# hucsmn/suffix_array

Hardware: AMD Instinct MI355X
Metric: input MB/s indexed (SA build) (higher is better)
Workload: dtype u8; 1 GPU; c3_english_256m: 268435456 bytes per GPU, seed base + rank, one independent text per GPU; n_bytes=268435456, sigma=57, symbols_per_key=13, refinement_rounds=9, text_rounds=0, radix_passes=25, unresolved_after_initial_sort=199000237

## Files before the change

### suffix_array_amd/csrc/host/pipeline.hpp

```cpp
#pragma once
#include "support.hpp"
#include "tuning.hpp"
#include "pool.hpp"
#include "sort.hpp"
#include "readback.hpp"

#include <functional>

namespace sa {

static inline Tuning env_tuning() { return Tuning::from_env(N_SORT_VARIANTS, N_SORT32_VARIANTS, N_OS_SHAPES64, N_OS_SHAPES32); }
static inline Tuning route_tuning()
{
    const Tuning tn = env_tuning();
    g_posted_off = tn.no_posted_readback;
    return tn;
}

constexpr size_t GRAM_MAX_ENTRIES = (size_t)1 << 24;
static_assert(GROUP_CAP_MAX == GS_CAP, "Tuning clamps SA_AMD_GROUP_CAP to the kernel's cap");

struct Workspace {
    uint64_t *keysA, *keysB, *keysC;
    uint32_t *valsA, *valsB, *isa, *U0, *U1, *G0, *G1;
// ... 154 lines not shown
                            const Tuning &tn, bool trace)
{
    KeyParams &P = *Pp;
    const uint64_t se = P.sigma;
    const uint64_t cap = (uint64_t)((size_t)n < GRAM_MAX_ENTRIES ? (size_t)n : GRAM_MAX_ENTRIES);
    int g = 0;
    uint64_t S = 1;
    for (int t = 1; t <= 8; ++t) {
        if (S * se > cap) break;
        S *= se; g = t;
        if (tn.gram_g >= 2 && g == tn.gram_g) break;
    }
    if (g < 2) return SA_AMD_OK;
    uint64_t top = 1;
    for (int t = 0; t + 1 < g; ++t) top *= se;
    const int64_t gtiles = ceil_div((int64_t)S, GT_TILE);
    HIP_TRY(hipMemsetAsync(w.gram_flags, 0, (size_t)S, st));
    PROF(KC_MISC, n, st, hipLaunchKernelGGL((k_gram_mark), dim3((unsigned)ceil_div(ceil_div(n, KB_TILE), GM_TPW)), dim3(KB_THREADS), 0, st, dT, n, P, g,
                                            (uint32_t)top, w.gram_flags));
    PROF(KC_MISC, (int64_t)S, st, hipLaunchKernelGGL((k_gram_count), dim3((unsigned)gtiles), dim3(GT_THREADS), 0, st,
                                            (const uint8_t *)w.gram_flags, (int64_t)S, w.tcnt));
    PROF(KC_RR_SCAN, gtiles, st, hipLaunchKernelGGL((k_rr_scan), dim3(1), dim3(SPINE_THREADS), 0, st, w.tcnt, w.thead, gtiles, w.total));
    uint32_t D = 0;
    { const int rcw = read_words(&D, w.total, 4, st); if (rcw) return rcw; }
    int m = 0;
    unsigned __int128 pw = 1;
    while (D >= 2 && (m + 1) * g <= 64 && pw * D <= ((unsigned __int128)1 << 64)) { pw *= D; ++m; }
    int tail = 0;
    while (m > 0 && tail < tn.gram_tail_max && m * g + tail + 1 <= 64 && pw * se <= ((unsigned __int128)1 << 64)) { pw *= se; ++tail; }
    const int gram_bits = m > 0 ? bit_length((uint64_t)(pw - 1)) : 0;
    const int plain_passes = (int)ceil_div(*key_bits, RADIX_BITS), gram_passes = (int)ceil_div(gram_bits, RADIX_BITS);
    const int syms = m * g + tail;
    const bool better = m > 0 && (syms > P.k || (syms == P.k && gram_passes < plain_passes));
    if (trace) fprintf(stderr, "suffix_array_amd: gram keys: %u of %llu %d-grams occur -> %d symbols (%d grams + %d plain) in %d bits (plain: %d in %d) -> %s\n",
                       D, (unsigned long long)S, g, syms, m, tail, gram_bits, P.k, *key_bits, better ? "gram keys" : "plain keys");
    if (!better) return SA_AMD_OK;
    PROF(KC_MISC, (int64_t)S, st, hipLaunchKernelGGL((k_gram_table), dim3((unsigned)gtiles), dim3(GT_THREADS), 0, st,
                                            (const uint8_t *)w.gram_flags, (int64_t)S, (const uint32_t *)w.tcnt, w.gram_table));
    P.gram = g; P.gram_m = m; P.gram_tail = tail; P.gram_top = (uint32_t)top; P.gram_D = D; P.gram_table = w.gram_table;
    P.bits = 0; P.k = syms; P.mask = ~0ull;
    *key_bits = gram_bits;
    return SA_AMD_OK;
}

struct EarlyDownload {
    int off = 0;
    int64_t threshold = 0;
    std::function<void(hipEvent_t)> start;
    std::function<int64_t()> stop;
    bool started = false;
    int64_t m_snap = 0;
    int64_t covered = 0;
    int64_t holes = 0;
    const uint32_t *d_bits = nullptr, *d_tile_off = nullptr, *d_holes = nullptr;
    hipEvent_t ev = nullptr;
};

struct DeviceBuild : BuildCore {
    EarlyDownload *early = nullptr;
    bool trace = false;
    double trace_t = 0;
    double lap() { const double t = now_ms(), d = t - trace_t; trace_t = t; return d; }
    bool timing_only() const
    {
#ifdef SA_AMD_DIAG
        return tn.timing_only_initial_sort;
#else
        return false;
#endif
    }
    KeyParams P, Ptext;
    int sigma = 0, key_bits = 0, top_shift = 0;
    bool force_dense = false, text_ok = false, probe_dense = false;
    SortResult<uint64_t> sr;
    const uint32_t *sorted32 = nullptr;
    int bucket_top_bits = 0;
    bool flat_text = false;
    bool bucket_finished = false;
    uint64_t *sorted0 = nullptr;
    int64_t tiles = 0, depth = 0;
    uint32_t m32 = 0;
    bool lists_ready = false, finished32 = false, fused64 = false, sparse = false;
    bool isa_tail_ranks = false;
    int s_sym = 0, tkb = 0;
    bool unary_done = false;
    RoundState rs;

    int early_maybe_start()
    {
        if (!early || early->started || L.m <= 0 || L.m > early->threshold || !early->start) return SA_AMD_OK;
        if (!early->ev && hipEventCreateWithFlags(&early->ev, hipEventDisableTiming) != hipSuccess) { (void)hipGetLastError(); return SA_AMD_OK; }
        hipLaunchKernelGGL(k_set_u32, dim3(1), dim3(1), 0, st, dSA, (uint32_t)n);
        LAUNCH_CHECK(st);
        HIP_TRY(hipMemsetAsync(w.early_bits, 0, (((size_t)n + 1 + 31) / 32 + EARLY_THREADS) * 4, st));
        int64_t blocks = ceil_div(L.m, 256 * 8);
        if (blocks > 65536) blocks = 65536;
        if ((((uintptr_t)L.U) & 15) != 0) return SA_AMD_OK;
        PROF(KC_MISC, L.m, st, hipLaunchKernelGGL((k_early_mark), dim3((unsigned)blocks), dim3(256), 0, st, (const uint32_t *)L.U, L.m, (uint32_t)early->off, w.early_bits));
        HIP_TRY(hipEventRecord(early->ev, st));
        early->started = true;
        early->m_snap = L.m;
        if (trace) fprintf(stderr, "suffix_array_amd: early download starts with %lld suffixes still tied\n", (long long)L.m);
        early->start(early->ev);
        return SA_AMD_OK;
    }
    int early_finish()
    {
        if (!early || !early->started) return SA_AMD_OK;
        early->covered = early->stop ? early->stop() : 0;
        if (early->covered > n + early->off) early->covered = n + early->off;
        early->holes = 0;
        if (early->covered <= 0) return SA_AMD_OK;
        const int64_t tiles_e = ceil_div(early->covered, EARLY_TILE);
        const int64_t words = ceil_div(early->covered, 32);
        PROF(KC_MISC, early->covered, st, hipLaunchKernelGGL((k_early_count), dim3((unsigned)tiles_e), dim3(EARLY_THREADS), 0, st,
                                                             (const uint32_t *)w.early_bits, words, w.early_cnt));
        PROF(KC_RR_SCAN, tiles_e, st, hipLaunchKernelGGL((k_rr_scan), dim3(1), dim3(SPINE_THREADS), 0, st, w.early_cnt, (uint32_t *)nullptr, tiles_e, w.early_cnt + tiles_e));
        uint32_t *holes = (uint32_t *)w.keysC;
        PROF(KC_MISC, early->covered, st, hipLaunchKernelGGL((k_early_gather), dim3((unsigned)tiles_e), dim3(EARLY_THREADS), 0, st,
                                                             (const uint32_t *)w.early_bits, words, (const uint32_t *)w.early_cnt,
                                                             (const uint32_t *)(dSA + 1 - early->off), holes));
        uint32_t total = 0;
        { const int rcw = read_words(&total, w.early_cnt + tiles_e, 4, st); if (rcw) return rcw; }
        early->holes = total;
        early->d_bits = w.early_bits; early->d_tile_off = w.early_cnt; early->d_holes = holes;
        return SA_AMD_OK;
    }

    int choose_bucket_bits() const
    {
        if (tn.no_bucket_sort || n < tn.bucket_min_n || n <= 1) return 0;
        const bool wide_ok = onesweep_on(w.ss, tn) && tn.onesweep32_shape == 0;
        if (tn.bucket_bits == 18 && wide_ok) return 18;
        if (tn.bucket_bits == 16) return 16;
        const bool value_bits = wide_ok && !tn.no_value_bits && !tn.no_text_keys && g_bits <= 30 &&
                                ((sigma == 256 && P.bits == 8) || (sigma == 4 && P.bits == 2 && !tn.no_packed_text));
        if (value_bits && (n >> 16) > 7500 && (n >> 18) * 10 <= bucket_cap_max() * 9) return 18;
        if ((n >> 16) * 10 <= bucket_cap(2) * 9) return 16;
        if (wide_ok && (n >> 18) * 10 <= bucket_cap_max() * 9) return 18;
        if ((n >> 16) * 10 <= bucket_cap_max() * 9) return 16;
        return 0;
    }

    bool flat_rule_applies() const { return n >= 2 && n < tn.top32_probe_min_n && n < ((int64_t)1 << 24) && !tn.no_flat_rule; }

    template <int ISA_MODE>
    int rr_apply_setup(const RrApply &a)
    {
        const uint64_t *k = sr.keys;
        if (head_flags)
            return isa_tail_ranks ? rr_apply<true, false, ISA_MODE, uint64_t, true, true>(k, a) : rr_apply<true, false, ISA_MODE, uint64_t, false, true>(k, a);
        return isa_tail_ranks ? rr_apply<true, false, ISA_MODE, uint64_t, true>(k, a) : rr_apply<true, false, ISA_MODE>(k, a);
    }
    int rebuild_sorted_keys()
    {
        if (!head_flags) return SA_AMD_OK;
        int64_t blocks = ceil_div(n, GK_THREADS);
        if (blocks > 65536) blocks = 65536;
        PROF(KC_GATHER, n, st, hipLaunchKernelGGL((k_keys_of_suffixes), dim3((unsigned)blocks), dim3(GK_THREADS), 0, st, dT, P, n, (const uint32_t *)SA, sr.keys));
        head_flags = nullptr;
        if (trace) fprintf(stderr, "suffix_array_amd: sorted keys rebuilt from the suffix array (the route taken reads them)\n");
        return SA_AMD_OK;
    }
    RrApply first_args(uint32_t n_text, uint32_t *has_isa = nullptr) const
    {
        RrApply a;
// ... 228 lines not shown

    int initial_sort()
    {
        int rc;
        sr.keys = w.keysA; sr.vals = w.valsA; sr.passes = 0;
        head_flags = nullptr;
        sorted32 = nullptr;
        bucket_finished = false;
        const bool iota = n >= 2 && key_bits > 0;
        uint32_t *vals0 = iota ? (uint32_t *)nullptr : w.valsA;
        uint8_t *packed_out = nullptr;
        if ((P.bits == 1 || P.bits == 2 || P.bits == 4) && n >= 64 && !tn.no_packed_text) {
            packed_out = w.packed;
            HIP_TRY(hipMemsetAsync(packed_out + (size_t)(n >> 3) * P.bits, 0, 64, st));
        }
        if (top_shift) {
            rc = initial_sort_top32(vals0, packed_out, iota);
            if (rc) return rc;
        } else {
            const FirstCounts fc = sort_first_counts(w.ss, tn, n, false);
            const bool counted = n > 1 && key_bits > 0;
            if (counted) HIP_TRY(hipMemsetAsync(fc.zero_ptr, 0, fc.zero_bytes, st));
            if ((rc = build_keys64(vals0, packed_out, fc, counted))) return rc;
            bool ss_done = false;
#ifdef SA_AMD_DIAG
            if (iota && counted && tn.sample_sort && n >= tn.sample_sort_min_n && key_bits > 32 && onesweep_on(w.ss, tn) && !timing_only()) {
                const size_t need_big = ((size_t)ceil_div(n, SS_TILE) + SS_WAYS) * SS_IDS2 * 4;
                if (need_big <= (size_t)n * 4 && (size_t)n * 4 >= ((size_t)4 << 20)) {
                    rc = sample_sort64(w.keysA, w.keysB, w.keysC, w.valsA, w.valsB, w.U0, w.U1, w.isa, w.G0, w.bk_start, SA, n, key_bits, w.ss, st, &local, tn,
                                       &ss_done, trace);
                    if (rc) return rc;
                    if (ss_done) { sr.keys = w.keysB; sr.vals = SA; sr.passes = 3; sr.skipped = 0; }
                    else {
                        HIP_TRY(hipMemsetAsync(fc.zero_ptr, 0, fc.zero_bytes, st));
                        if ((rc = build_keys64(vals0, packed_out, fc, true))) return rc;
                    }
                }
            }
#endif
            if (!ss_done) {
            const bool dense_expected = force_dense || probe_dense || !text_ok;
            const bool want_flags = tn.head_flags != 0 && (tn.head_flags == 2 || dense_expected) && flags_slab_ok && onesweep_on(w.ss, tn) && !timing_only() &&
                                    !tn.fused64 && n >= 2 && key_bits > 0;
            SortJob<uint64_t> job{ w.keysA, w.valsA, w.keysB, w.valsB, n, 0, key_bits };
            job.final_vals = SA;
            job.iota = iota; job.may_skip = sigma == 1; job.first_counted = counted;
            job.head_flags = want_flags ? (uint8_t *)w.keysC : (uint8_t *)nullptr;
            rc = sort_pairs(job, w.ss, st, tn, &sr, &local);
            if (rc) return rc;
            if (want_flags && sr.passes > 0 && sr.vals == SA) head_flags = (uint8_t *)w.keysC;
            if (trace && head_flags) fprintf(stderr, "suffix_array_amd: initial sort: the last pass wrote group-start flags, not the sorted keys\n");
            }
        }
        P.packed = packed_out;
        if (sr.vals != SA) {
            PROF(KC_MISC, n, st, hipLaunchKernelGGL((k_copy_u32), dim3(1), dim3(256), 0, st, sr.vals, SA, n));
        }

        return SA_AMD_OK;
    }

    int first_round_from_sorted_keys()
    {
        int rc;
        L.U = w.U0; L.Un = w.U1; L.G = w.G0; L.Gn = w.G1;
        L.V = w.valsA;
        tiles = ceil_div(n, RR_TILE);
        m32 = 0;
        L.m = 0;
        L.rkA = w.keysA; L.rkB = w.keysB;
        sorted0 = sr.keys;
        lists_ready = false;
        depth = P.k;
        Ptext = P;
        if (P.bits == 0) Ptext.bits = bit_length(P.sigma - 1);
        Ptext.gram = 0;
        s_sym = 0; tkb = 0;
        {
            const int room = 64 - g_bits;
            s_sym = room / Ptext.bits;
            if (s_sym > 64) s_sym = 64;
            tkb = s_sym * Ptext.bits;
        }
        finished32 = false; fused64 = false;
        if (top_shift && rs.local_ok && !tn.no_fused_finish && !timing_only()) {
            const int cap = tn.group_cap;
            uint32_t *surv_bits = w.surv_bits, *surv_head = w.isa;
            if (!bucket_finished) {
            if ((rc = zero_finish_records())) return rc;
            KeySrc K = KeySrc(); K.mode = KS_LOWKEY; K.kb = top_shift;
            PROF(KC_FINISH, n, st, hipLaunchKernelGGL((k_finish_sorted<uint32_t, KS_LOWKEY, false>), dim3((unsigned)ceil_div(n, FT_TILE)), dim3(FT_THREADS),
                                                     0, st, sorted32, SA, dT, P, n, K, cap, surv_bits, surv_head, w.tcnt, w.total, (uint32_t *)nullptr,
                                                     (uint32_t *)nullptr, (uint32_t *)nullptr));
            }
            if (!bucket_finished) PROF(KC_RR_SCAN, tiles, st, hipLaunchKernelGGL((k_rr_scan), dim3(1), dim3(SPINE_THREADS), 0, st, w.tcnt, w.thead, tiles, w.total));
            uint32_t words[ROUND_WORDS];
            { const int rcw = read_words(words, w.total, sizeof(words), st); if (rcw) return rcw; }
            const uint32_t tied64 = bucket_finished ? (uint32_t)chg_sum(words, 1) : words[0], unowned = words[1], tied32 = (uint32_t)chg_sum(words);
            if (bucket_finished && tied64 != 0 && unowned == 0)
                PROF(KC_RR_SCAN, tiles, st, hipLaunchKernelGGL((k_rr_scan), dim3(1), dim3(SPINE_THREADS), 0, st, w.tcnt, w.thead, tiles, w.total));
            if (unowned == 0) {
                finished32 = true;
                L.m = tied64;
                local.locally_sorted += tied32;
                local.unresolved_after_initial = L.m;
                if (L.m > 0) {
                    PROF(KC_RR_APPLY, n, st, hipLaunchKernelGGL((k_surv_compact), dim3((unsigned)tiles), dim3(256), 0, st, (const uint32_t *)surv_bits,
                                                                (const uint32_t *)surv_head, (const uint32_t *)SA, n, (const uint32_t *)w.tcnt,
                                                                (const uint32_t *)w.total, L.U, L.G, L.V));
                    L.keys_beside(w, sr.keys);
                    lists_ready = true;
                }
            }
        }
        if (!top_shift && text_ok && rs.local_ok && s_sym > 0 && tn.fused64 && !tn.no_fused_finish && !tn.sparse_div_set && !timing_only()) {
            const int cap = tn.group_cap;
            const int64_t ft_tiles = ceil_div(n, FT_TILE);
            uint32_t *surv_head = w.isa;
            HIP_TRY(hipMemsetAsync(w.surv_bits, 0, ((size_t)n + 31) / 32 * 4, st));
            HIP_TRY(hipMemsetAsync(w.todo_bits, 0, ((size_t)n + 31) / 32 * 4, st));
            HIP_TRY(hipMemsetAsync(w.ft_cnt, 0, (size_t)(ft_tiles + 1) * 4, st));
            HIP_TRY(hipMemsetAsync(w.ft_head, 0, (size_t)(ft_tiles + 1) * 4, st));
            HIP_TRY(hipMemsetAsync(w.surv_cnt, 0, (size_t)tiles * 4, st));
            HIP_TRY(hipMemsetAsync(w.thead, 0, (size_t)tiles * 4, st));
            HIP_TRY(hipMemsetAsync(w.total, 0, 32, st));
            HIP_TRY(hipMemsetAsync(w.chg, 0, (size_t)RR_CHG_COUNTERS * 32 * 4, st));
            KeySrc K = KeySrc(); K.mode = KS_TEXT; K.h = depth; K.s = s_sym; K.kb = tkb;
            PROF(KC_FINISH, n, st, hipLaunchKernelGGL((k_finish_sorted<uint64_t, KS_TEXT, true>), dim3((unsigned)ft_tiles), dim3(FT_THREADS), 0, st,
                                                     (const uint64_t *)sorted0, SA, dT, Ptext, n, K, cap, w.surv_bits, surv_head, w.surv_cnt, w.total,
                                                     w.todo_bits, w.ft_cnt, w.ft_head));
            PROF(KC_RR_SCAN, ft_tiles, st, hipLaunchKernelGGL((k_rr_scan), dim3(1), dim3(SPINE_THREADS), 0, st, w.ft_cnt, w.ft_head, ft_tiles, w.total + 3));
            uint32_t words[ROUND_WORDS];
            { const int rcw = read_words(words, w.total, sizeof(words), st); if (rcw) return rcw; }
            const int64_t tied0 = (uint32_t)chg_sum(words), m_todo = words[3];
            local.unresolved_after_initial = tied0;
            local.locally_sorted += tied0 - m_todo;
            L.keys_beside(w, sr.keys);
            if (m_todo > 0) {
                PROF(KC_RR_APPLY, n, st, hipLaunchKernelGGL((k_todo_compact<uint64_t>), dim3((unsigned)ft_tiles), dim3(FT_THREADS), 0, st,
                                                            (const uint64_t *)sorted0, (const uint32_t *)SA, n, (const uint32_t *)w.todo_bits,
                                                            (const uint32_t *)w.ft_cnt, (const uint32_t *)w.ft_head, (const uint32_t *)(w.total + 3),
                                                            L.U, L.G, L.V));
                L.m = m_todo;
                RoundState own;
                own.local_ok = true;
                RefineRound round(*this, Ptext, K, own);
                if ((rc = round.run<NO_RERANK>())) return rc;
                const Refined &rf = round.rf;
                if ((rc = rr_count<false>(rf.keys, L.U, L.m, nullptr, 0, nullptr, w.ft_cnt, w.ft_head))) return rc;
                if ((rc = rr_scan(L.m, w.ft_cnt, w.ft_head, w.total + 4))) return rc;
                RrApply a = round_args(rf);
                a.tile_cnt = w.ft_cnt; a.tile_head = w.ft_head; a.tile_total = w.total + 4;
                a.has_isa = w.surv_bits; a.pair_v = w.surv_cnt;
                if ((rc = rr_apply<false, true, 4>(rf.keys, a))) return rc;
            }
            PROF(KC_RR_SCAN, tiles, st, hipLaunchKernelGGL((k_rr_scan), dim3(1), dim3(SPINE_THREADS), 0, st, w.surv_cnt, w.thead, tiles, w.total));
            { const int rcw = read_words(&m32, w.total, 4, st); if (rcw) return rcw; }
            L.m = m32;
            L.U = w.U0; L.G = w.G0; L.V = w.valsA; L.Un = w.U1; L.Gn = w.G1;
            if (L.m > 0)
                PROF(KC_RR_APPLY, n, st, hipLaunchKernelGGL((k_surv_compact), dim3((unsigned)tiles), dim3(256), 0, st, (const uint32_t *)w.surv_bits,
                                                            (const uint32_t *)surv_head, (const uint32_t *)SA, n, (const uint32_t *)w.surv_cnt,
                                                            (const uint32_t *)w.total, L.U, L.G, L.V));
            fused64 = true;
            lists_ready = true;
            depth += s_sym;
            local.text_rounds++;
            local.rounds++;
            if (trace) fprintf(stderr, "suffix_array_amd: text round %d depth %lld: tied %lld -> %lld  (%.2f ms)\n", local.text_rounds, (long long)depth, (long long)tied0, (long long)L.m, lap());
        }
        return SA_AMD_OK;
    }

    int group_heads()
    {
        int rc;
        if (!finished32 && !fused64) {
        rc = top_shift ? rr_count<true, uint32_t>(sorted32, nullptr, n)
           : head_flags ? rr_count<true, uint64_t, true, true>((const uint64_t *)sr.keys, nullptr, n, w.tnext)
                        : rr_count<true, uint64_t, true>((const uint64_t *)sr.keys, nullptr, n, w.tnext);
        if (rc) return rc;
        if ((rc = rr_scan(n))) return rc;
        { const int rcw = read_words(&m32, w.total, 4, st); if (rcw) return rcw; }
        L.m = m32;
        local.unresolved_after_initial = L.m;
        if (timing_only()) L.m = 0;
        }
        return SA_AMD_OK;
    }

    int finish_top32_ties()
    {
        int rc;
        if (!finished32 && top_shift && L.m > 0) {
            L.keys_beside(w, sr.keys);
            if ((rc = rr_apply<true, false, 1, uint32_t>(sorted32, first_args(0u, w.has_isa)))) return rc;
            KeySrc K = KeySrc(); K.mode = KS_LOWKEY; K.kb = top_shift;
            RefineRound round(*this, P, K, rs);
            if ((rc = round.run<NO_RERANK>())) return rc;
            const Refined &rf = round.rf;
            if ((rc = rr_count<false>(rf.keys, L.U, L.m))) return rc;
            if ((rc = rr_scan(L.m))) return rc;
            if ((rc = rr_apply<false, true, 3>(rf.keys, round_args(rf)))) return rc;
            { const int rcw = read_words(&m32, w.total, 4, st); if (rcw) return rcw; }
            L.m = m32;
            L.advance(rf);
            lists_ready = true;
            local.unresolved_after_initial = L.m;
        }
        return SA_AMD_OK;
    }

    int rank_setup_and_text_rounds()
    {
        int rc;
        key2_bits = bit_length((uint64_t)(2 * n));
        const int64_t sparse_div = tn.sparse_div;
        const int64_t sparse_limit = n / sparse_div;
        sparse = false;
        const bool dense_first = L.m > 0 && !lists_ready && (force_dense || (!text_ok && L.m > sparse_limit) || (probe_dense && L.m > sparse_limit));
        if (L.m > 0 && dense_first) {
            isa_tail_ranks = !tn.no_first_tail;
            if (isa_tail_ranks)
                PROF(KC_RR_SCAN, tiles, st, hipLaunchKernelGGL((k_rr_scan_next), dim3(1), dim3(SPINE_THREADS), 0, st, w.tnext, tiles, (uint32_t *)nullptr));
            RrApply a = first_args((uint32_t)n);
            a.tile_next = isa_tail_ranks ? w.tnext : (uint32_t *)nullptr;
            if (binned(n, n, tn)) {
                uint64_t *pk = (sr.keys == w.keysA) ? w.keysB : w.keysA;
                const bool from_sa = !tn.setup_key_copy && (((uintptr_t)dSA) & 15) == 0;
                const size_t H = ((size_t)n + 1 + 3) & ~(size_t)3;
                uint32_t *pk32 = (uint32_t *)pk, *sk32 = (uint32_t *)sr.keys;
                uint64_t *pk_out = from_sa ? (uint64_t *)nullptr : pk;
                uint32_t *pv_out = from_sa ? pk32 + H + 1 : w.U1;
                a.pair_k = pk_out; a.pair_v = pv_out;
                if ((rc = rr_apply_setup<2>(a))) return rc;
                if (from_sa) {
                    hipLaunchKernelGGL(k_set_u32, dim3(1), dim3(1), 0, st, dSA, (uint32_t)n);
                    LAUNCH_CHECK(st);
                    rc = scatter_binned(w.ss, w.isa, dSA, pk32 + H, sk32, sk32 + H, n + 1, n, st, &local, tn, false, pk32);
                } else
                    rc = scatter_binned(w.ss, w.isa, (uint32_t *)pk, w.U1, (uint32_t *)sr.keys, w.G1, n, n, st, &local, tn);
                if (rc) return rc;
            } else if ((rc = rr_apply_setup<0>(a))) return rc;
        } else if (L.m > 0) {
            if ((rc = rebuild_sorted_keys())) return rc;
            HIP_TRY(hipMemsetAsync(w.has_isa, 0, ((size_t)n + 31) / 32 * 4, st));
            if (!lists_ready) {
                L.keys_beside(w, sr.keys);
                if ((rc = rr_apply<true, false, 1>((const uint64_t *)sorted0, first_args(0u, w.has_isa)))) return rc;
            }
            bool progressing = true;
            while (text_ok && s_sym > 0 && L.m > sparse_limit && local.text_rounds < tn.max_text_rounds && progressing) {
                if ((rc = early_maybe_start())) return rc;
                const int64_t m_before = L.m;
                KeySrc K = KeySrc(); K.mode = KS_TEXT; K.h = depth; K.s = s_sym; K.kb = tkb;
                RefineRound round(*this, Ptext, K, rs, rs.prev_clean && rs.local_ok && !tn.no_defer);
                if ((rc = round.run<3>())) return rc;
                after_round(round);
                depth += s_sym;
                local.text_rounds++;
                progressing = L.m * 4 <= m_before * 3;
                if (trace) fprintf(stderr, "suffix_array_amd: text round %d depth %lld: tied %lld -> %lld  (%.2f ms)\n", local.text_rounds, (long long)depth, (long long)m_before, (long long)L.m, lap());
            }
            if (L.m > sparse_limit) {
                int64_t blocks = ceil_div(n, 256);
                if (blocks > 16384) blocks = 16384;
                if (binned(n, n, tn) && (((uintptr_t)dSA) & 15) == 0) {
                    hipLaunchKernelGGL(k_set_u32, dim3(1), dim3(1), 0, st, dSA, (uint32_t)n);
                    LAUNCH_CHECK(st);
                    const size_t H = ((size_t)n + 1 + 3) & ~(size_t)3;
                    rc = scatter_binned(w.ss, w.isa, dSA, nullptr, (uint32_t *)L.rkB, (uint32_t *)L.rkB + H, n + 1, n, st, &local, tn, true,
                                        (uint32_t *)L.rkA, (uint32_t *)L.rkA + H);
                    if (rc) return rc;
                } else
                    PROF(KC_SCATTER, n, st, hipLaunchKernelGGL((k_isa_from_sa), dim3((unsigned)blocks), dim3(256), 0, st, (const uint32_t *)SA, w.isa, n));
                blocks = ceil_div(L.m, 256);
                if (blocks > 16384) blocks = 16384;
                PROF(KC_SCATTER, L.m, st, hipLaunchKernelGGL((k_isa_tied), dim3((unsigned)blocks), dim3(256), 0, st, (const uint32_t *)L.V,
                                                           (const uint32_t *)L.G, w.isa, L.m, n));
            } else {
                sparse = L.m > 0;
            }
        }
        local.sparse_mode = sparse ? 1 : 0;
        if (trace) fprintf(stderr, "suffix_array_amd: initial sort + text rounds + rank set-up done, %lld tied (%.2f ms since the last line)\n", (long long)L.m, lap());
        return SA_AMD_OK;
    }

    int doubling_rounds()
    {
        int rc;
        const int64_t depth_text = depth;
        int64_t h = depth;
        rs.parent_tail = isa_tail_ranks;
        rs.changed_prev = isa_tail_ranks ? L.m : 0;
        rs.m_local_off = L.m;
        rs.counters_clear = false;
        while (L.m > 0) {
            if (local.rounds >= 48) return SA_AMD_EINTERNAL;
            if ((rc = early_maybe_start())) return rc;
            const int64_t m_before = L.m;
            KeySrc K = KeySrc();
            K.mode = sparse ? KS_SPARSE : KS_RANK; K.h = h; K.kb = key2_bits; K.isa = w.isa;
            K.has_isa = w.has_isa; K.sorted_keys = sorted0; K.sorted_top32 = sorted32; K.sa = SA; K.depth = depth_text; K.top_shift = top_shift;
            if (!rs.local_ok && !tn.no_local_sort && L.m * 2 < rs.m_local_off) rs.local_ok = true;
            const bool retry_local = !rs.local_ok && ++rs.rounds_local_off >= 3;
// ... 100 lines not shown
```

### suffix_array_amd/csrc/kernels/rerank.hpp

```cpp
#pragma once
#include "common.hpp"

namespace sa {

constexpr int RR_THREADS = 1024;
constexpr int RR_ITEMS = 8;
constexpr int RR_TILE = RR_THREADS * RR_ITEMS;

constexpr int RR_WAVE_ELEMS = WAVE * RR_ITEMS;

struct WaveGroups { uint64_t head[RR_ITEMS], tied[RR_ITEMS], valid[RR_ITEMS], phead[RR_ITEMS]; };

template <typename KeyT, bool PARENTS = false>
__device__ __forceinline__ WaveGroups rr_wave_classify(const KeyT *__restrict__ keys, int64_t m, int64_t wbase, int key_shift, int g_shift = 0,
                                                       uint64_t *kout = nullptr)
{
    const int l = lane_id();
    uint64_t k[RR_ITEMS];
    WaveGroups g;
#pragma unroll
    for (int r = 0; r < RR_ITEMS; ++r) {
        const int64_t i = wbase + 64 * r + l;
        k[r] = i < m ? ((uint64_t)keys[i] >> key_shift) : 0ull;
        g.valid[r] = __ballot(i < m);
    }
    const uint64_t before = (wbase > 0 && wbase - 1 < m) ? ((uint64_t)keys[wbase - 1] >> key_shift) : 0ull;
    const uint64_t after = (wbase + RR_WAVE_ELEMS < m) ? ((uint64_t)keys[wbase + RR_WAVE_ELEMS] >> key_shift) : 0ull;
#pragma unroll
    for (int r = 0; r < RR_ITEMS; ++r) {
        uint64_t up = shfl64(k[r], l ? l - 1 : 0);
        const uint64_t prev_last = r ? shfl64(k[r ? r - 1 : 0], 63) : before;
        if (l == 0) up = prev_last;
        const int64_t i = wbase + 64 * r + l;
        g.head[r] = __ballot(i < m && (i == 0 || k[r] != up));
        g.phead[r] = PARENTS ? __ballot(i < m && (i == 0 || ((k[r] ^ up) >> g_shift) != 0ull)) : 0ull;
    }
    if (kout) {
#pragma unroll
        for (int r = 0; r < RR_ITEMS; ++r) kout[r] = k[r];
        kout[RR_ITEMS] = before;
    }
    const uint64_t last_key = shfl64(k[RR_ITEMS - 1], 63);
    const bool boundary_after = (wbase + RR_WAVE_ELEMS >= m) || after != last_key;
#pragma unroll
    for (int r = 0; r < RR_ITEMS; ++r) {
        const uint64_t bnd = g.head[r] | ~g.valid[r];
        const uint64_t bnd_next0 = (r + 1 < RR_ITEMS) ? ((g.head[(r + 1) % RR_ITEMS] | ~g.valid[(r + 1) % RR_ITEMS]) & 1ull)
                                                      : (boundary_after ? 1ull : 0ull);
        const uint64_t next = (bnd >> 1) | (bnd_next0 << 63);
        g.tied[r] = g.valid[r] & ~(g.head[r] & next);
    }
    return g;
}

struct WaveBytes { uint2 w; uint32_t fa; };
__device__ __forceinline__ WaveBytes rr_wave_load_bytes(const uint8_t *__restrict__ bytes, int64_t m, int64_t wbase, uint8_t none)
{
    const int64_t i0 = wbase + 8 * lane_id();
    const int64_t a = wbase + RR_WAVE_ELEMS;
    WaveBytes b;
    b.w = i0 < m ? *(const uint2 *)(bytes + i0) : make_uint2(0u, 0u);
    b.fa = a < m ? (uint32_t)bytes[a] : (uint32_t)none;
    return b;
}

template <bool PARENTS = false>
__device__ __forceinline__ WaveGroups rr_wave_classify_flags(const WaveBytes &raw, const uint64_t *__restrict__ keys, int64_t m, int64_t wbase)
{
    const int l = lane_id();
    WaveGroups g;
    const int64_t i0 = wbase + 8 * l;
    const int64_t a = wbase + RR_WAVE_ELEMS;
    const uint32_t fa = raw.fa;
    uint32_t hb = 0;
    if (i0 < m) {
        const uint2 w = raw.w;
        hb = (((w.x & 0x01010101u) * 0x01020408u) >> 24 & 15u) | ((((w.y & 0x01010101u) * 0x01020408u) >> 24 & 15u) << 4);
        if ((w.x | w.y) & 0x02020202u) {
#pragma unroll
            for (int k = 0; k < 8; ++k) {
                const uint32_t f = ((k < 4 ? w.x : w.y) >> (8 * (k & 3))) & 255u;
                if (f == OS_HF_SEAM && i0 + k < m && i0 + k > 0 && keys[i0 + k] != keys[i0 + k - 1]) hb |= 1u << k;
            }
        }
        if (i0 == 0) hb |= 1u;
        if (i0 + 8 > m) hb &= (1u << (int)(m - i0)) - 1u;
    }
    const uint32_t h1 = (uint32_t)__shfl_down((int)hb, 1, WAVE), h2 = (uint32_t)__shfl_down((int)hb, 2, WAVE), h3 = (uint32_t)__shfl_down((int)hb, 3, WAVE);
    const uint32_t quad = hb | (h1 << 8) | (h2 << 16) | (h3 << 24);
    const int64_t left = m - wbase;
#pragma unroll
    for (int r = 0; r < RR_ITEMS; ++r) {
        const uint32_t lo = (uint32_t)__builtin_amdgcn_readlane((int)quad, 8 * r), hi = (uint32_t)__builtin_amdgcn_readlane((int)quad, 8 * r + 4);
        const int64_t here = left - 64 * r;
        g.valid[r] = here >= 64 ? ~0ull : (here <= 0 ? 0ull : ((1ull << here) - 1ull));
        g.head[r] = (((uint64_t)hi << 32) | lo) & g.valid[r];
        g.phead[r] = PARENTS ? g.head[r] : 0ull;
    }
    const bool boundary_after = fa == OS_HF_START || (fa == OS_HF_SEAM && keys[a] != keys[a - 1]);
#pragma unroll
    for (int r = 0; r < RR_ITEMS; ++r) {
        const uint64_t bnd = g.head[r] | ~g.valid[r];
        const uint64_t bnd_next0 = (r + 1 < RR_ITEMS) ? ((g.head[(r + 1) % RR_ITEMS] | ~g.valid[(r + 1) % RR_ITEMS]) & 1ull)
                                                      : (boundary_after ? 1ull : 0ull);
        const uint64_t next = (bnd >> 1) | (bnd_next0 << 63);
        g.tied[r] = g.valid[r] & ~(g.head[r] & next);
    }
    return g;
}

template <bool PARENTS = false>
__device__ __forceinline__ WaveGroups rr_wave_classify_flags(const uint8_t *__restrict__ flags, const uint64_t *__restrict__ keys, int64_t m, int64_t wbase)
{
    return rr_wave_classify_flags<PARENTS>(rr_wave_load_bytes(flags, m, wbase, OS_HF_START), keys, m, wbase);
}

template <bool PARENTS = false>
__device__ __forceinline__ WaveGroups rr_wave_classify_status(const WaveBytes &raw, const uint64_t *__restrict__ keys, int64_t m, int64_t wbase_in)
{
    const int l = lane_id();
    WaveGroups g;
    const int64_t wbase = ((int64_t)__builtin_amdgcn_readfirstlane((int)(wbase_in >> 32)) << 32) | (uint32_t)__builtin_amdgcn_readfirstlane((int)(uint32_t)wbase_in);
    const int64_t i0 = wbase + 8 * l;
    const int64_t a = wbase + RR_WAVE_ELEMS;
    const uint32_t fa = raw.fa;
    uint32_t hb = 0, pb = 0;
    if (i0 < m) {
        const uint2 w = raw.w;
        auto plane = [&](int b) -> uint32_t {
            return ((((w.x >> b) & 0x01010101u) * 0x01020408u) >> 24 & 15u) | (((((w.y >> b) & 0x01010101u) * 0x01020408u) >> 24 & 15u) << 4);
        };
        const uint32_t here = i0 + 8 > m ? (1u << (int)(m - i0)) - 1u : 255u;
        pb = plane(3) & here;
        const uint32_t kd = plane(1) & here;
        hb = pb | (plane(2) & ~kd & here);
        const uint32_t need = kd & ~pb;
        if (need) {
            uint64_t k[8];
            if (i0 + 8 <= m) {
                const uint4 *src = (const uint4 *)(keys + i0);
#pragma unroll
                for (int q = 0; q < 4; ++q) {
                    const uint4 x = src[q];
                    k[2 * q] = ((uint64_t)x.y << 32) | x.x;
                    k[2 * q + 1] = ((uint64_t)x.w << 32) | x.z;
                }
            } else {
#pragma unroll
                for (int q = 0; q < 8; ++q) k[q] = i0 + q < m ? keys[i0 + q] : 0ull;
            }
            const uint64_t before = ((need & 1u) && i0 > 0) ? keys[i0 - 1] : ~k[0];
            uint32_t ne = before != k[0] ? 1u : 0u;
#pragma unroll
            for (int q = 1; q < 8; ++q) ne |= (k[q] != k[q - 1] ? 1u : 0u) << q;
            hb |= need & ne;
        }
    }
    const uint32_t h1 = (uint32_t)__shfl_down((int)hb, 1, WAVE), h2 = (uint32_t)__shfl_down((int)hb, 2, WAVE), h3 = (uint32_t)__shfl_down((int)hb, 3, WAVE);
    const uint32_t quad = hb | (h1 << 8) | (h2 << 16) | (h3 << 24);
    uint32_t pquad = 0;
    if (PARENTS) {
        const uint32_t p1 = (uint32_t)__shfl_down((int)pb, 1, WAVE), p2 = (uint32_t)__shfl_down((int)pb, 2, WAVE), p3 = (uint32_t)__shfl_down((int)pb, 3, WAVE);
        pquad = pb | (p1 << 8) | (p2 << 16) | (p3 << 24);
    }
    const int64_t left = m - wbase;
#pragma unroll
    for (int r = 0; r < RR_ITEMS; ++r) {
        const uint32_t lo = (uint32_t)__builtin_amdgcn_readlane((int)quad, 8 * r), hi = (uint32_t)__builtin_amdgcn_readlane((int)quad, 8 * r + 4);
        const int64_t here = left - 64 * r;
        g.valid[r] = here >= 64 ? ~0ull : (here <= 0 ? 0ull : ((1ull << here) - 1ull));
        g.head[r] = (((uint64_t)hi << 32) | lo) & g.valid[r];
        g.phead[r] = 0ull;
        if (PARENTS) {
            const uint32_t plo = (uint32_t)__builtin_amdgcn_readlane((int)pquad, 8 * r), phi = (uint32_t)__builtin_amdgcn_readlane((int)pquad, 8 * r + 4);
            g.phead[r] = (((uint64_t)phi << 32) | plo) & g.valid[r];
        }
    }
    const bool boundary_after = (fa & RS_PHEAD) != 0 || ((fa & RS_KEYED) ? keys[a] != keys[a - 1] : (fa & RS_HEAD) != 0);
#pragma unroll
    for (int r = 0; r < RR_ITEMS; ++r) {
        const uint64_t bnd = g.head[r] | ~g.valid[r];
        const uint64_t bnd_next0 = (r + 1 < RR_ITEMS) ? ((g.head[(r + 1) % RR_ITEMS] | ~g.valid[(r + 1) % RR_ITEMS]) & 1ull)
                                                      : (boundary_after ? 1ull : 0ull);
        const uint64_t next = (bnd >> 1) | (bnd_next0 << 63);
        g.tied[r] = g.valid[r] & ~(g.head[r] & next);
    }
    return g;
}

template <bool PARENTS = false>
__device__ __forceinline__ WaveGroups rr_wave_classify_status(const uint8_t *__restrict__ status, const uint64_t *__restrict__ keys, int64_t m, int64_t wbase)
{
    return rr_wave_classify_status<PARENTS>(rr_wave_load_bytes(status, m, wbase, RS_PHEAD), keys, m, wbase);
}

constexpr uint32_t RR_NO_HEAD = 0xffffffffu;
constexpr int RR_CHG_COUNTERS = 16;
__device__ __forceinline__ uint32_t rr_first_head_code(const WaveGroups &g, int64_t wbase, int r_from)
{
    uint32_t code = RR_NO_HEAD;
#pragma unroll
    for (int r = RR_ITEMS - 1; r >= 0; --r) {
        if (r >= r_from && g.head[r]) {
            const int b = __builtin_ctzll(g.head[r]);
            code = ((uint32_t)(wbase + 64 * r + b) << 1) | (uint32_t)((g.phead[r] >> b) & 1ull);
        }
    }
    return code;
}

constexpr int RR_COUNT_SPAN = 4;
static_assert(RR_COUNT_SPAN <= RR_THREADS / WAVE, "wave s of the workgroup reduces tile s of the span");
template <bool BYTES> constexpr int rr_count_span() { return BYTES ? RR_COUNT_SPAN : 1; }

__device__ __forceinline__ void rr_reduce16(uint32_t &a, uint32_t &b, uint32_t &c)
{
    static_assert(RR_THREADS / WAVE == 16, "one lane per wave of the tile");
#pragma unroll
    for (int o = 8; o > 0; o >>= 1) {
        const uint32_t ta = (uint32_t)__shfl_xor((int)a, o, WAVE), tb = (uint32_t)__shfl_xor((int)b, o, WAVE), tc = (uint32_t)__shfl_xor((int)c, o, WAVE);
        a += ta; b = b > tb ? b : tb; c = c < tc ? c : tc;
    }
}

template <bool FIRST, typename KeyT = uint64_t, bool PARENTS = false, bool FLAGS = false>
__global__ __launch_bounds__(RR_THREADS) __attribute__((amdgpu_waves_per_eu(8))) void k_rr_count(const KeyT *__restrict__ keys,
                                                          const uint32_t *__restrict__ U, int64_t m,
                                                          uint32_t *__restrict__ tile_cnt,
                                                          uint32_t *__restrict__ tile_head, int key_shift,
                                                          uint32_t *__restrict__ tile_first, int g_shift,
                                                          const uint32_t *__restrict__ gate = nullptr,
                                                          const uint8_t *__restrict__ head_flags = nullptr)
{
    static_assert(!FLAGS || (sizeof(KeyT) == 8 && (FIRST || PARENTS)), "group-start flags come from the 64-bit initial sort, status bytes from a dense round");
    constexpr int SPAN = rr_count_span<FLAGS>();
    constexpr int NW = RR_THREADS / WAVE;
    __shared__ uint32_t wcnt[SPAN][NW], whead[SPAN][NW], wfirst[SPAN][NW];
    if (gate && *gate) return;
#ifdef SA_AMD_DIAG
    const bool stamping = g_rr_stamp_on != 0 && threadIdx.x == 0;
    unsigned long long t_prev = stamping ? __builtin_amdgcn_s_memtime() : 0ull, t_phase[4] = { 0ull, 0ull, 0ull, 0ull };
    auto stamp = [&](int phase, bool wait) {
        if (stamping) {
            if (wait) __builtin_amdgcn_s_waitcnt(0);
            const unsigned long long now = __builtin_amdgcn_s_memtime();
            t_phase[phase] = now - t_prev;
            t_prev = now;
            if (phase == 3)
                for (int p = 0; p < 4; ++p) atomicAdd(&g_phase_cycles[p], t_phase[p]);
        }
    };
#else
    auto stamp = [](int, bool) {};
#endif
    const int w = __builtin_amdgcn_readfirstlane(wave_id());
    const int64_t tiles = (m + RR_TILE - 1) / RR_TILE;
    const int64_t tile0 = (int64_t)blockIdx.x * SPAN;
    WaveBytes raw[SPAN];
    if constexpr (FLAGS) {
#pragma unroll
        for (int s = 0; s < SPAN; ++s)
            raw[s] = rr_wave_load_bytes(head_flags, m, (tile0 + s) * RR_TILE + (int64_t)w * RR_WAVE_ELEMS, FIRST ? OS_HF_START : RS_PHEAD);
    }
    stamp(0, false);
#pragma unroll
    for (int s = 0; s < SPAN; ++s) {
    const int64_t wbase = (tile0 + s) * RR_TILE + (int64_t)w * RR_WAVE_ELEMS;
    uint64_t kk[RR_ITEMS + 1];
    WaveGroups g;
    if constexpr (FLAGS && FIRST) g = rr_wave_classify_flags<false>(raw[s], (const uint64_t *)keys, m, wbase);
    else if constexpr (FLAGS) g = rr_wave_classify_status<true>(raw[s], (const uint64_t *)keys, m, wbase);
    else g = rr_wave_classify<KeyT, false>(keys, m, wbase, key_shift, 0, PARENTS ? kk : nullptr);
    uint32_t cnt = 0, lasthead = 0;
#pragma unroll
    for (int r = 0; r < RR_ITEMS; ++r) {
        cnt += (uint32_t)__popcll(g.tied[r]);
        if (g.head[r]) lasthead = (uint32_t)(wbase + 64 * r + (63 - __builtin_clzll(g.head[r]))) + 1u;
    }
    uint32_t first_code = RR_NO_HEAD;
    if constexpr (PARENTS && FLAGS && !FIRST) first_code = rr_first_head_code(g, wbase, 0);
    else if (PARENTS) {
        bool found = false;
#pragma unroll
        for (int r = 0; r < RR_ITEMS; ++r) {
            if (!found && g.head[r]) {
                found = true;
                const int b = __builtin_ctzll(g.head[r]);
                const int64_t i = wbase + 64 * r + b;
                if constexpr (FLAGS) first_code = ((uint32_t)i << 1) | 1u;
                else {
                const uint64_t mine = shfl64(kk[r], b);
                const uint64_t left = b ? shfl64(kk[r], b - 1) : (r ? shfl64(kk[r ? r - 1 : 0], 63) : kk[RR_ITEMS]);
                const uint32_t ph = (i == 0 || ((mine ^ left) >> g_shift) != 0ull) ? 1u : 0u;
                first_code = ((uint32_t)i << 1) | ph;
                }
            }
        }
    }
    if (lane_id() == 0) { wcnt[s][w] = cnt; whead[s][w] = lasthead; wfirst[s][w] = first_code; }
    }
    stamp(1, true);
    __syncthreads();
    stamp(2, true);
    if (w < SPAN && tile0 + w < tiles) {
        const int l = lane_id();
        uint32_t tot = l < NW ? wcnt[w][l] : 0u, mx = l < NW ? whead[w][l] : 0u, fc = l < NW ? wfirst[w][l] : RR_NO_HEAD;
        rr_reduce16(tot, mx, fc);
        if (l == 0) {
            tile_cnt[tile0 + w] = tot;
            tile_head[tile0 + w] = (FIRST || mx == 0u) ? mx : U[mx - 1u] + 1u;
            if (PARENTS) tile_first[tile0 + w] = fc;
        }
    }
    stamp(3, true);
}
template <bool BYTES> inline unsigned rr_count_grid(int64_t m) { return (unsigned)(((m + RR_TILE - 1) / RR_TILE + rr_count_span<BYTES>() - 1) / rr_count_span<BYTES>()); }

__device__ __forceinline__ void rr_scan_next_body(uint32_t *__restrict__ tile_first, int64_t tiles, uint32_t *__restrict__ changed_cnt)
{
    __shared__ uint32_t s_min[SPINE_THREADS];
    const int t = threadIdx.x;
    const int64_t per = (tiles + SPINE_THREADS - 1) / SPINE_THREADS;
    int64_t b = (int64_t)t * per, e = b + per;
    if (b > tiles) b = tiles;
    if (e > tiles) e = tiles;
    uint32_t mn = RR_NO_HEAD;
    for (int64_t i = b; i < e; ++i) { const uint32_t c = tile_first[i]; mn = mn < c ? mn : c; }
    s_min[t] = mn;
    __syncthreads();
    for (int o = 1; o < SPINE_THREADS; o <<= 1) {
        const uint32_t other = t + o < SPINE_THREADS ? s_min[t + o] : RR_NO_HEAD;
        __syncthreads();
        if (other < s_min[t]) s_min[t] = other;
        __syncthreads();
    }
    uint32_t run = t + 1 < SPINE_THREADS ? s_min[t + 1] : RR_NO_HEAD;
    for (int64_t i = e - 1; i >= b; --i) {
        const uint32_t c = tile_first[i];
        tile_first[i] = run;
        run = run < c ? run : c;
    }
    if (t < RR_CHG_COUNTERS && changed_cnt) changed_cnt[t * 32] = 0u;
}

__global__ __launch_bounds__(SPINE_THREADS) void k_rr_scan_next(uint32_t *__restrict__ tile_first, int64_t tiles, uint32_t *__restrict__ changed_cnt)
{
    rr_scan_next_body(tile_first, tiles, changed_cnt);
}

__device__ __forceinline__ void rr_scan_body(uint32_t *__restrict__ tile_cnt, uint32_t *__restrict__ tile_head, int64_t tiles,
                                             uint32_t *__restrict__ out_total)
{
    __shared__ uint32_t lds[SPINE_THREADS / WAVE + 1];
    const int64_t per = ((tiles + SPINE_THREADS - 1) / SPINE_THREADS + 3) & ~(int64_t)3;
    int64_t b = (int64_t)threadIdx.x * per, e = b + per;
    if (b > tiles) b = tiles;
    if (e > tiles) e = tiles;
    const int64_t ev = b + ((e - b) & ~(int64_t)3);
    const bool heads = tile_head != nullptr;
    uint32_t s = 0, mx = 0;
    for (int64_t i = b; i < ev; i += 4) {
        const uint4 c = *(const uint4 *)(tile_cnt + i);
        s += c.x + c.y + c.z + c.w;
        if (heads) { const uint4 h = *(const uint4 *)(tile_head + i); mx = max(max(mx, max(h.x, h.y)), max(h.z, h.w)); }
    }
    for (int64_t i = ev; i < e; ++i) { s += tile_cnt[i]; if (heads) mx = max(mx, tile_head[i]); }
    uint32_t tot, mtot;
    uint32_t off = block_excl_sum<SPINE_THREADS>(s, lds, &tot);
    uint32_t incm = block_incl_max<SPINE_THREADS>(mx, lds, &mtot);
    uint32_t prevm = __shfl_up(incm, 1, WAVE);
    __shared__ uint32_t wlast[SPINE_THREADS / WAVE];
    if (lane_id() == WAVE - 1) wlast[wave_id()] = incm;
    __syncthreads();
    if (lane_id() == 0) prevm = wave_id() ? wlast[wave_id() - 1] : 0u;
    uint32_t run = prevm;
    for (int64_t i = b; i < ev; i += 4) {
        const uint4 c = *(const uint4 *)(tile_cnt + i);
        uint4 oc;
        oc.x = off; off += c.x; oc.y = off; off += c.y; oc.z = off; off += c.z; oc.w = off; off += c.w;
        *(uint4 *)(tile_cnt + i) = oc;
// ... 198 lines not shown
```

Baseline: 6093 MB/s.

## Count tied groups from per-lane bits and fuse tile-next scan into group-head scan

For the flag/status paths of the rerank count kernel, tied counts, last head and first head code are now computed straight from each lane's 8-bit head/valid masks using ballots. This replaces the full wave transpose into 64-bit WaveGroups words. On the dense-first host path, the separate k_rr_scan_next launch is dropped by running a two-block k_rr_scan_round that also produces the tile-next scan during group_heads. It removes shuffles and readlanes in the count kernel plus one small kernel launch, at the cost of added host state and a condition that must match the later dense_first decision.

```diff
diff --git a/suffix_array_amd/csrc/host/pipeline.hpp b/suffix_array_amd/csrc/host/pipeline.hpp
--- a/suffix_array_amd/csrc/host/pipeline.hpp
+++ b/suffix_array_amd/csrc/host/pipeline.hpp
@@ -260,6 +260,7 @@
     uint32_t m32 = 0;
     bool lists_ready = false, finished32 = false, fused64 = false, sparse = false;
     bool isa_tail_ranks = false;
+    bool tnext_scanned = false;
     int s_sym = 0, tkb = 0;
     bool unary_done = false;
     RoundState rs;
@@ -654,7 +655,7 @@
             if (s_sym > 64) s_sym = 64;
             tkb = s_sym * Ptext.bits;
         }
-        finished32 = false; fused64 = false;
+        finished32 = false; fused64 = false; tnext_scanned = false;
         if (top_shift && rs.local_ok && !tn.no_fused_finish && !timing_only()) {
             const int cap = tn.group_cap;
             uint32_t *surv_bits = w.surv_bits, *surv_head = w.isa;
@@ -752,7 +753,11 @@
            : head_flags ? rr_count<true, uint64_t, true, true>((const uint64_t *)sr.keys, nullptr, n, w.tnext)
                         : rr_count<true, uint64_t, true>((const uint64_t *)sr.keys, nullptr, n, w.tnext);
         if (rc) return rc;
-        if ((rc = rr_scan(n))) return rc;
+        tnext_scanned = !top_shift && (force_dense || probe_dense || !text_ok);
+        if (tnext_scanned)
+            PROF(KC_RR_SCAN, tiles, st, hipLaunchKernelGGL((k_rr_scan_round), dim3(2), dim3(SPINE_THREADS), 0, st, w.tcnt, w.thead, tiles, w.total, w.tnext,
+                                                           (uint32_t *)nullptr, (uint32_t *)nullptr, (const uint32_t *)nullptr));
+        else if ((rc = rr_scan(n))) return rc;
         { const int rcw = read_words(&m32, w.total, 4, st); if (rcw) return rcw; }
         L.m = m32;
         local.unresolved_after_initial = L.m;
@@ -793,7 +798,7 @@
         const bool dense_first = L.m > 0 && !lists_ready && (force_dense || (!text_ok && L.m > sparse_limit) || (probe_dense && L.m > sparse_limit));
         if (L.m > 0 && dense_first) {
             isa_tail_ranks = !tn.no_first_tail;
-            if (isa_tail_ranks)
+            if (isa_tail_ranks && !tnext_scanned)
                 PROF(KC_RR_SCAN, tiles, st, hipLaunchKernelGGL((k_rr_scan_next), dim3(1), dim3(SPINE_THREADS), 0, st, w.tnext, tiles, (uint32_t *)nullptr));
             RrApply a = first_args((uint32_t)n);
             a.tile_next = isa_tail_ranks ? w.tnext : (uint32_t *)nullptr;
diff --git a/suffix_array_amd/csrc/kernels/rerank.hpp b/suffix_array_amd/csrc/kernels/rerank.hpp
--- a/suffix_array_amd/csrc/kernels/rerank.hpp
+++ b/suffix_array_amd/csrc/kernels/rerank.hpp
@@ -64,15 +64,16 @@
     return b;
 }
 
-template <bool PARENTS = false>
-__device__ __forceinline__ WaveGroups rr_wave_classify_flags(const WaveBytes &raw, const uint64_t *__restrict__ keys, int64_t m, int64_t wbase)
-{
-    const int l = lane_id();
-    WaveGroups g;
-    const int64_t i0 = wbase + 8 * l;
+struct LaneBits { uint32_t hb, pb, vb; bool after; };
+
+__device__ __forceinline__ LaneBits rr_lane_bits_flags(const WaveBytes &raw, const uint64_t *__restrict__ keys, int64_t m, int64_t wbase)
+{
+    const int64_t i0 = wbase + 8 * lane_id();
     const int64_t a = wbase + RR_WAVE_ELEMS;
     const uint32_t fa = raw.fa;
+    LaneBits x;
     uint32_t hb = 0;
+    x.vb = 0;
     if (i0 < m) {
         const uint2 w = raw.w;
         hb = (((w.x & 0x01010101u) * 0x01020408u) >> 24 & 15u) | ((((w.y & 0x01010101u) * 0x01020408u) >> 24 & 15u) << 4);
@@ -84,53 +85,29 @@
             }
         }
         if (i0 == 0) hb |= 1u;
-        if (i0 + 8 > m) hb &= (1u << (int)(m - i0)) - 1u;
-    }
-    const uint32_t h1 = (uint32_t)__shfl_down((int)hb, 1, WAVE), h2 = (uint32_t)__shfl_down((int)hb, 2, WAVE), h3 = (uint32_t)__shfl_down((int)hb, 3, WAVE);
-    const uint32_t quad = hb | (h1 << 8) | (h2 << 16) | (h3 << 24);
-    const int64_t left = m - wbase;
-#pragma unroll
-    for (int r = 0; r < RR_ITEMS; ++r) {
-        const uint32_t lo = (uint32_t)__builtin_amdgcn_readlane((int)quad, 8 * r), hi = (uint32_t)__builtin_amdgcn_readlane((int)quad, 8 * r + 4);
-        const int64_t here = left - 64 * r;
-        g.valid[r] = here >= 64 ? ~0ull : (here <= 0 ? 0ull : ((1ull << here) - 1ull));
-        g.head[r] = (((uint64_t)hi << 32) | lo) & g.valid[r];
-        g.phead[r] = PARENTS ? g.head[r] : 0ull;
-    }
-    const bool boundary_after = fa == OS_HF_START || (fa == OS_HF_SEAM && keys[a] != keys[a - 1]);
-#pragma unroll
-    for (int r = 0; r < RR_ITEMS; ++r) {
-        const uint64_t bnd = g.head[r] | ~g.valid[r];
-        const uint64_t bnd_next0 = (r + 1 < RR_ITEMS) ? ((g.head[(r + 1) % RR_ITEMS] | ~g.valid[(r + 1) % RR_ITEMS]) & 1ull)
-                                                      : (boundary_after ? 1ull : 0ull);
-        const uint64_t next = (bnd >> 1) | (bnd_next0 << 63);
-        g.tied[r] = g.valid[r] & ~(g.head[r] & next);
-    }
-    return g;
-}
-
-template <bool PARENTS = false>
-__device__ __forceinline__ WaveGroups rr_wave_classify_flags(const uint8_t *__restrict__ flags, const uint64_t *__restrict__ keys, int64_t m, int64_t wbase)
-{
-    return rr_wave_classify_flags<PARENTS>(rr_wave_load_bytes(flags, m, wbase, OS_HF_START), keys, m, wbase);
-}
-
-template <bool PARENTS = false>
-__device__ __forceinline__ WaveGroups rr_wave_classify_status(const WaveBytes &raw, const uint64_t *__restrict__ keys, int64_t m, int64_t wbase_in)
-{
-    const int l = lane_id();
-    WaveGroups g;
-    const int64_t wbase = ((int64_t)__builtin_amdgcn_readfirstlane((int)(wbase_in >> 32)) << 32) | (uint32_t)__builtin_amdgcn_readfirstlane((int)(uint32_t)wbase_in);
-    const int64_t i0 = wbase + 8 * l;
+        x.vb = i0 + 8 > m ? (1u << (int)(m - i0)) - 1u : 255u;
+        hb &= x.vb;
+    }
+    x.hb = hb; x.pb = hb;
+    x.after = fa == OS_HF_START || (fa == OS_HF_SEAM && keys[a] != keys[a - 1]);
+    return x;
+}
+
+__device__ __forceinline__ LaneBits rr_lane_bits_status(const WaveBytes &raw, const uint64_t *__restrict__ keys, int64_t m, int64_t wbase)
+{
+    const int64_t i0 = wbase + 8 * lane_id();
     const int64_t a = wbase + RR_WAVE_ELEMS;
     const uint32_t fa = raw.fa;
+    LaneBits x;
     uint32_t hb = 0, pb = 0;
+    x.vb = 0;
     if (i0 < m) {
         const uint2 w = raw.w;
         auto plane = [&](int b) -> uint32_t {
             return ((((w.x >> b) & 0x01010101u) * 0x01020408u) >> 24 & 15u) | (((((w.y >> b) & 0x01010101u) * 0x01020408u) >> 24 & 15u) << 4);
         };
         const uint32_t here = i0 + 8 > m ? (1u << (int)(m - i0)) - 1u : 255u;
+        x.vb = here;
         pb = plane(3) & here;
         const uint32_t kd = plane(1) & here;
         hb = pb | (plane(2) & ~kd & here);
@@ -141,9 +118,9 @@
                 const uint4 *src = (const uint4 *)(keys + i0);
 #pragma unroll
                 for (int q = 0; q < 4; ++q) {
-                    const uint4 x = src[q];
-                    k[2 * q] = ((uint64_t)x.y << 32) | x.x;
-                    k[2 * q + 1] = ((uint64_t)x.w << 32) | x.z;
+                    const uint4 x4 = src[q];
+                    k[2 * q] = ((uint64_t)x4.y << 32) | x4.x;
+                    k[2 * q + 1] = ((uint64_t)x4.w << 32) | x4.z;
                 }
             } else {
 #pragma unroll
@@ -156,10 +133,20 @@
             hb |= need & ne;
         }
     }
+    x.hb = hb; x.pb = pb;
+    x.after = (fa & RS_PHEAD) != 0 || ((fa & RS_KEYED) ? keys[a] != keys[a - 1] : (fa & RS_HEAD) != 0);
+    return x;
+}
+
+template <bool PARENTS, bool OWN_P>
+__device__ __forceinline__ WaveGroups rr_wave_transpose(const LaneBits &x, int64_t m, int64_t wbase)
+{
+    WaveGroups g;
+    const uint32_t hb = x.hb, pb = x.pb;
     const uint32_t h1 = (uint32_t)__shfl_down((int)hb, 1, WAVE), h2 = (uint32_t)__shfl_down((int)hb, 2, WAVE), h3 = (uint32_t)__shfl_down((int)hb, 3, WAVE);
     const uint32_t quad = hb | (h1 << 8) | (h2 << 16) | (h3 << 24);
     uint32_t pquad = 0;
-    if (PARENTS) {
+    if (PARENTS && OWN_P) {
         const uint32_t p1 = (uint32_t)__shfl_down((int)pb, 1, WAVE), p2 = (uint32_t)__shfl_down((int)pb, 2, WAVE), p3 = (uint32_t)__shfl_down((int)pb, 3, WAVE);
         pquad = pb | (p1 << 8) | (p2 << 16) | (p3 << 24);
     }
@@ -170,13 +157,13 @@
         const int64_t here = left - 64 * r;
         g.valid[r] = here >= 64 ? ~0ull : (here <= 0 ? 0ull : ((1ull << here) - 1ull));
         g.head[r] = (((uint64_t)hi << 32) | lo) & g.valid[r];
-        g.phead[r] = 0ull;
-        if (PARENTS) {
+        g.phead[r] = (PARENTS && !OWN_P) ? g.head[r] : 0ull;
+        if (PARENTS && OWN_P) {
             const uint32_t plo = (uint32_t)__builtin_amdgcn_readlane((int)pquad, 8 * r), phi = (uint32_t)__builtin_amdgcn_readlane((int)pquad, 8 * r + 4);
             g.phead[r] = (((uint64_t)phi << 32) | plo) & g.valid[r];
         }
     }
-    const bool boundary_after = (fa & RS_PHEAD) != 0 || ((fa & RS_KEYED) ? keys[a] != keys[a - 1] : (fa & RS_HEAD) != 0);
+    const bool boundary_after = x.after;
 #pragma unroll
     for (int r = 0; r < RR_ITEMS; ++r) {
         const uint64_t bnd = g.head[r] | ~g.valid[r];
@@ -188,10 +175,22 @@
     return g;
 }
 
+__device__ __forceinline__ int64_t rr_uniform(int64_t v)
+{
+    return ((int64_t)__builtin_amdgcn_readfirstlane((int)(v >> 32)) << 32) | (uint32_t)__builtin_amdgcn_readfirstlane((int)(uint32_t)v);
+}
+
 template <bool PARENTS = false>
-__device__ __forceinline__ WaveGroups rr_wave_classify_status(const uint8_t *__restrict__ status, const uint64_t *__restrict__ keys, int64_t m, int64_t wbase)
-{
-    return rr_wave_classify_status<PARENTS>(rr_wave_load_bytes(status, m, wbase, RS_PHEAD), keys, m, wbase);
+__device__ __forceinline__ WaveGroups rr_wave_classify_flags(const uint8_t *__restrict__ flags, const uint64_t *__restrict__ keys, int64_t m, int64_t wbase)
+{
+    return rr_wave_transpose<PARENTS, false>(rr_lane_bits_flags(rr_wave_load_bytes(flags, m, wbase, OS_HF_START), keys, m, wbase), m, wbase);
+}
+
+template <bool PARENTS = false>
+__device__ __forceinline__ WaveGroups rr_wave_classify_status(const uint8_t *__restrict__ status, const uint64_t *__restrict__ keys, int64_t m, int64_t wbase_in)
+{
+    const int64_t wbase = rr_uniform(wbase_in);
+    return rr_wave_transpose<PARENTS, true>(rr_lane_bits_status(rr_wave_load_bytes(status, m, wbase, RS_PHEAD), keys, m, wbase), m, wbase);
 }
 
 constexpr uint32_t RR_NO_HEAD = 0xffffffffu;
@@ -207,6 +206,30 @@
         }
     }
     return code;
+}
+
+struct WaveCount { uint32_t cnt, lasthead, first_code; };
+__device__ __forceinline__ WaveCount rr_wave_count_bits(const LaneBits &x, int64_t wbase)
+{
+    const uint32_t b = (x.hb | ~x.vb) & 255u;
+    uint32_t nb = (uint32_t)__shfl_down((int)b, 1, WAVE) & 1u;
+    if (lane_id() == WAVE - 1) nb = x.after ? 1u : 0u;
+    const uint32_t tied = x.vb & ~(x.hb & ((b >> 1) | (nb << 7)));
+    WaveCount c;
+    c.cnt = 0;
+#pragma unroll
+    for (int k = 0; k < RR_ITEMS; ++k) c.cnt += (uint32_t)__popcll(__ballot((tied >> k) & 1u));
+    c.lasthead = 0; c.first_code = RR_NO_HEAD;
+    const uint64_t any = __ballot(x.hb != 0);
+    if (any) {
+        const int top = 63 - __builtin_clzll(any), low = __builtin_ctzll(any);
+        const uint32_t ht = (uint32_t)__builtin_amdgcn_readlane((int)x.hb, top);
+        const uint32_t hl = (uint32_t)__builtin_amdgcn_readlane((int)x.hb, low), pl = (uint32_t)__builtin_amdgcn_readlane((int)x.pb, low);
+        c.lasthead = (uint32_t)(wbase + 8 * top + (31 - __builtin_clz(ht))) + 1u;
+        const int k = __builtin_ctz(hl);
+        c.first_code = ((uint32_t)(wbase + 8 * low + k) << 1) | ((pl >> k) & 1u);
+    }
+    return c;
 }
 
 constexpr int RR_COUNT_SPAN = 4;
@@ -266,20 +289,25 @@
 #pragma unroll
     for (int s = 0; s < SPAN; ++s) {
     const int64_t wbase = (tile0 + s) * RR_TILE + (int64_t)w * RR_WAVE_ELEMS;
+    uint32_t cnt = 0, lasthead = 0;
+    uint32_t first_code = RR_NO_HEAD;
+    if constexpr (FLAGS) {
+        const int64_t wb = rr_uniform(wbase);
+        LaneBits x;
+        if constexpr (FIRST) x = rr_lane_bits_flags(raw[s], (const uint64_t *)keys, m, wb);
+        else x = rr_lane_bits_status(raw[s], (const uint64_t *)keys, m, wb);
+        const WaveCount c = rr_wave_count_bits(x, wb);
+        cnt = c.cnt; lasthead = c.lasthead;
+        if (PARENTS) first_code = c.first_code;
+    } else {
     uint64_t kk[RR_ITEMS + 1];
-    WaveGroups g;
-    if constexpr (FLAGS && FIRST) g = rr_wave_classify_flags<false>(raw[s], (const uint64_t *)keys, m, wbase);
-    else if constexpr (FLAGS) g = rr_wave_classify_status<true>(raw[s], (const uint64_t *)keys, m, wbase);
-    else g = rr_wave_classify<KeyT, false>(keys, m, wbase, key_shift, 0, PARENTS ? kk : nullptr);
-    uint32_t cnt = 0, lasthead = 0;
+    const WaveGroups g = rr_wave_classify<KeyT, false>(keys, m, wbase, key_shift, 0, PARENTS ? kk : nullptr);
 #pragma unroll
     for (int r = 0; r < RR_ITEMS; ++r) {
         cnt += (uint32_t)__popcll(g.tied[r]);
         if (g.head[r]) lasthead = (uint32_t)(wbase + 64 * r + (63 - __builtin_clzll(g.head[r]))) + 1u;
     }
-    uint32_t first_code = RR_NO_HEAD;
-    if constexpr (PARENTS && FLAGS && !FIRST) first_code = rr_first_head_code(g, wbase, 0);
-    else if (PARENTS) {
+    if (PARENTS) {
         bool found = false;
 #pragma unroll
         for (int r = 0; r < RR_ITEMS; ++r) {
@@ -287,15 +315,13 @@
                 found = true;
                 const int b = __builtin_ctzll(g.head[r]);
                 const int64_t i = wbase + 64 * r + b;
-                if constexpr (FLAGS) first_code = ((uint32_t)i << 1) | 1u;
-                else {
                 const uint64_t mine = shfl64(kk[r], b);
                 const uint64_t left = b ? shfl64(kk[r], b - 1) : (r ? shfl64(kk[r ? r - 1 : 0], 63) : kk[RR_ITEMS]);
                 const uint32_t ph = (i == 0 || ((mine ^ left) >> g_shift) != 0ull) ? 1u : 0u;
                 first_code = ((uint32_t)i << 1) | ph;
-                }
             }
         }
+    }
     }
     if (lane_id() == 0) { wcnt[s][w] = cnt; whead[s][w] = lasthead; wfirst[s][w] = first_code; }
     }
```

After: 6165 MB/s, median of 6. +1.2%, better.
